# mstksg/tensor-ops

Hardware: AMD Instinct MI355X
Metric: gradTOp steps/sec (ffLayer MNIST 784->256->10) + gmul TFLOP/s vs roofline (higher is better)
Workload: dtype f32

## Files before the change

tensor-ops_amd/csrc/gemm_small.hip:

```cpp
#include "common.hpp"

namespace to {

typedef float f32x16 __attribute__((ext_vector_type(16)));

template <class S>
struct SmallArgsT {
  const S* A;
  const S* B;
  S* C;
  const S* Cin;
  int M, N, K;
  long a_sm, a_sk, b_sk, b_sn, c_sm;
  long a_sb, b_sb, c_sb;
  int a_vec, b_vec;
  unsigned a_bytes, b_bytes;
  int tiles_n;
  int tiles_m;
  int tile_order;
  int kper;
  S alpha, beta;
  const S* bias;
  const S* dact;
  int act;
  int dact_kind;
  S* rowsum;
  const S* rowsum_in;
  S rowsum_alpha;
  int rowsum_acc;
  int loss_rows;
  const S* target;
  S* loss_out;
  const S* tail_w;
// ... 6 lines not shown
};

#ifdef TOPS_AB_KNOBS
#define SM_STAMP(i) do { if (stamp_on) g.dbg[i] = wall_clock64(); } while (0)
#else
#define SM_STAMP(i) do { } while (0)
#endif


template <class G>
__device__ __forceinline__ void tile_of(const G& g, int bid, int& tile_m, int& tile_n) {
  if (g.tile_order) {
    const int T = g.tiles_m * g.tiles_n, x = bid & 7, q = T >> 3, r = T & 7;
    bid = (x < r ? x * (q + 1) : r * (q + 1) + (x - r) * q) + (bid >> 3);
  }
  if (g.tile_order == 2) {
    tile_n = bid / g.tiles_m;
    tile_m = bid - tile_n * g.tiles_m;
  } else {
    tile_m = bid / g.tiles_n;
    tile_n = bid - tile_m * g.tiles_n;
  }
}

__device__ __forceinline__ float tanh_s(float x) { return tanhf(x); }
__device__ __forceinline__ double tanh_s(double x) { return tanh(x); }
__device__ __forceinline__ float exp_s(float x) { return expf(x); }
__device__ __forceinline__ double exp_s(double x) { return exp(x); }
__device__ __forceinline__ float log_s(float x) { return logf(x); }
__device__ __forceinline__ double log_s(double x) { return log(x); }
__device__ __forceinline__ float max_s(float a, float b) { return fmaxf(a, b); }
__device__ __forceinline__ double max_s(double a, double b) { return fmax(a, b); }

template <class S, int AMODE, int BMODE, int NW, int TS, int ONESHOT = 0, bool EXT = false>
__device__ __forceinline__ void gemm_small_body(const SmallArgsT<S>& g, const int bid, const long bz, S* ext_lds = nullptr,
                                                const int tid_in = -1) {
  constexpr int ES = (int)sizeof(S);
  static_assert(ES == 4 || TS == 16, "the fp64 matrix instruction is 16x16x4");
  constexpr int KG = (TS == 32) ? 2 : 4;
  constexpr int NR = (TS == 32) ? 16 : 4;
  constexpr int CK = 4 * KG;
  typedef S accv __attribute__((ext_vector_type(NR)));
  S (*red)[NR][64];
  S (*rsum)[64];
  S* dzs;
  if constexpr (EXT) {
    red = reinterpret_cast<S (*)[NR][64]>(ext_lds);
    rsum = reinterpret_cast<S (*)[64]>(ext_lds + NW * NR * 64);
    dzs = ext_lds + NW * NR * 64 + NW * 64;
  } else {
    __shared__ S red_s[NW][NR][64];
    __shared__ S rsum_s[NW][64];
    __shared__ S dzs_s[TS == 16 ? 16 * 17 : 1];
    red = red_s;
    rsum = rsum_s;
    dzs = dzs_s;
  }
  const int tid = tid_in >= 0 ? tid_in : (int)threadIdx.x, lane = tid & 63, wave = tid >> 6;
  const int l31 = lane & (TS - 1), half = lane / TS;
#ifdef TOPS_AB_KNOBS
  const bool stamp_on = g.dbg && bid == 0 && tid == 0;
#endif
  SM_STAMP(0);
  int tile_m, tile_n;
  tile_of(g, bid, tile_m, tile_n);
  const long m = (long)tile_m * TS + l31, n = (long)tile_n * TS + l31;
  const bool mv = m < g.M, nv = n < g.N;
// ... 38 lines not shown
      d[0] = __hiloint2double((int)v.y, (int)v.x); d[1] = __hiloint2double((int)v.w, (int)v.z);
      d[2] = __hiloint2double((int)w.y, (int)w.x); d[3] = __hiloint2double((int)w.w, (int)w.z);
    }
  };
  auto load_stage = [&](S (&a)[ST][4], S (&b)[ST][4], int k0) {
#pragma unroll
    for (int c = 0; c < ST; ++c) {
      const int kb = k0 + CK * c + 4 * half;
      if (AMODE == 0 && g.a_vec) {
        ld4(ra, mv & (kb < kend), a_base + kb * ES, a[c]);
      } else {
#pragma unroll
        for (int j = 0; j < 4; ++j) a[c][j] = ld1(ra, sel(mv & (kb + j < kend), a_base + (kb + j) * a_sk4));
      }
      if (BMODE == 1 && g.b_vec) {
        ld4(rb, nv & (kb < kend), b_base + kb * ES, b[c]);
      } else {
#pragma unroll
        for (int j = 0; j < 4; ++j) b[c][j] = ld1(rb, sel(nv & (kb + j < kend), b_base + (kb + j) * b_sk4));
      }
    }
  };
  auto mma_stage = [&](const S (&a)[ST][4], const S (&b)[ST][4]) {
#pragma unroll
    for (int c = 0; c < ST; ++c)
#pragma unroll
      for (int j = 0; j < 4; ++j) {
        if constexpr (ES == 8) acc = __builtin_amdgcn_mfma_f64_16x16x4f64(a[c][j], b[c][j], acc, 0, 0, 0);
        else if constexpr (TS == 32) acc = __builtin_amdgcn_mfma_f32_32x32x2f32(a[c][j], b[c][j], acc, 0, 0, 0);
        else acc = __builtin_amdgcn_mfma_f32_16x16x4f32(a[c][j], b[c][j], acc, 0, 0, 0);
        asum += a[c][j];
      }
  };
  auto row16 = [&](int kg, int r) { return ES == 8 ? kg + 4 * r : 4 * kg + r; };
  constexpr int NRW = (NR + NW - 1) / NW;
  S* Cb = g.C + bz * g.c_sb;
  const S* Ci = g.Cin ? g.Cin + bz * g.c_sb : nullptr;
  const S* Hd = g.dact ? g.dact + bz * g.c_sb : nullptr;
  S pf_ci[NRW], pf_hd[NRW], pf_bias = S(0);
  {
    const long col = (long)tile_n * TS + l31;
    if (g.bias && col < g.N) pf_bias = g.bias[col];
#pragma unroll
    for (int i = 0; i < NRW; ++i) {
      const int r = wave + i * NW;
      const int lrow = (TS == 32) ? (r & 3) + 8 * (r >> 2) + 4 * half : row16(half, r);
      const long row = (long)tile_m * TS + lrow;
      const bool ok = r < NR && row < g.M && col < g.N;
      pf_ci[i] = (Ci && ok) ? Ci[row * g.c_sm + col] : S(0);
      pf_hd[i] = (Hd && ok) ? Hd[row * g.c_sm + col] : S(0);
    }
  }
  constexpr int SK = CK * ST;
  SM_STAMP(1);
  if constexpr (ONESHOT) {
    if (kbeg < kend) {
      load_stage(a0, b0, kbeg);
#ifdef TOPS_AB_KNOBS
      if (stamp_on) { SM_STAMP(2); __builtin_amdgcn_s_waitcnt(0x0F70); SM_STAMP(3); }
#endif
      mma_stage(a0, b0);
    }
  } else {
    S a1[ST][4], b1[ST][4];
    if (kbeg < kend) load_stage(a0, b0, kbeg);
    for (int k0 = kbeg; k0 < kend; k0 += 2 * SK) {
      if (k0 + SK < kend) load_stage(a1, b1, k0 + SK);
      mma_stage(a0, b0);
      if (k0 + SK < kend) {
        if (k0 + 2 * SK < kend) load_stage(a0, b0, k0 + 2 * SK);
        mma_stage(a1, b1);
      }
    }
  }

  S tl_bw[2][4], tl_hv[2][4];
  if constexpr (TS == 16) {
    if (g.loss_rows && g.tail_out) {
      const int l15 = lane & 15, kg = lane >> 4;
      const int ntiles = (g.tail_n + 15) / 16;
#pragma unroll
      for (int u = 0; u < 2; ++u) {
        const int t = wave + u * NW;
        const long col = (long)t * 16 + l15;
        const bool cv = t < ntiles && col < g.tail_n;
#pragma unroll
        for (int st = 0; st < 4; ++st) {
          const int k = 4 * st + kg;
          tl_bw[u][st] = (cv && k < g.N) ? g.tail_w[(long)k * g.tail_n + col] : S(0);
        }
#pragma unroll
        for (int r = 0; r < 4; ++r) {
          const long row = (long)tile_m * 16 + row16(kg, r);
          tl_hv[u][r] = (cv && row < g.M) ? g.tail_h[row * g.tail_n + col] : S(0);
// ... 91 lines not shown
        if (4 * st < g.N) {
          const S a = dzs[l15 * 17 + 4 * st + kg];
#pragma unroll
          for (int u = 0; u < 2; ++u) {
            if constexpr (ES == 8) acc2[u] = __builtin_amdgcn_mfma_f64_16x16x4f64(a, tl_bw[u][st], acc2[u], 0, 0, 0);
            else acc2[u] = __builtin_amdgcn_mfma_f32_16x16x4f32(a, tl_bw[u][st], acc2[u], 0, 0, 0);
          }
        }
      }
#pragma unroll
      for (int u = 0; u < 2; ++u) {
        const int t = wave + u * NW;
        const long col = (long)t * 16 + l15;
#pragma unroll
        for (int r = 0; r < 4; ++r) {
          const long row = (long)tile_m * 16 + row16(kg, r);
          if (t < ntiles && row < g.M && col < g.tail_n)
            g.tail_out[row * g.tail_n + col] = acc2[u][r] * tl_hv[u][r] * (S(1) - tl_hv[u][r]);
        }
      }
      SM_STAMP(7);
    }
  }
#ifdef TOPS_AB_KNOBS
  if (stamp_on) { __builtin_amdgcn_s_waitcnt(0); SM_STAMP(8); }
#endif
}

template <class S, int AMODE, int BMODE, int NW, int TS, int ONESHOT = 0>
__global__ __launch_bounds__(NW * 64) void gemm_small_kernel(SmallArgsT<S> g) {
  gemm_small_body<S, AMODE, BMODE, NW, TS, ONESHOT>(g, (int)blockIdx.x, (long)blockIdx.z);
}

template <class S, int A1, int B1, int NW1, int TS1, int OS1, int A2, int B2, int NW2, int TS2, int OS2>
__global__ __launch_bounds__((NW1 > NW2 ? NW1 : NW2) * 64) void gemm_small_pair_kernel(SmallArgsT<S> g1,
                                                                                         SmallArgsT<S> g2, int n1) {
  if ((int)blockIdx.x < n1) {
    if (NW1 < NW2 && (int)(threadIdx.x >> 6) >= NW1) return;
    gemm_small_body<S, A1, B1, NW1, TS1, OS1>(g1, (int)blockIdx.x, 0);
  } else {
    if (NW2 < NW1 && (int)(threadIdx.x >> 6) >= NW2) return;
    gemm_small_body<S, A2, B2, NW2, TS2, OS2>(g2, (int)blockIdx.x - n1, 0);
  }
}

struct ChainSync {
  unsigned* ctr;
  int* status;
  long long timeout;
  int dev;
};

__device__ __forceinline__ bool chain_barrier(const ChainSync& cs, int which, unsigned epoch) {
  __shared__ int ok;
  if (cs.dev == 1) {
    __syncthreads();
    return true;
  }
  if (cs.dev != 2) __builtin_amdgcn_fence(__ATOMIC_RELEASE, "agent");
  if (threadIdx.x == 0) ok = 1;
  __syncthreads();
  unsigned* flags = cs.ctr + which * 256;
  if (threadIdx.x == 0) __hip_atomic_store(flags + blockIdx.x, epoch, __ATOMIC_RELEASE, __HIP_MEMORY_SCOPE_AGENT);
  if (threadIdx.x < gridDim.x) {
    const long long t0 = wall_clock64();
    while (__hip_atomic_load(flags + threadIdx.x, __ATOMIC_RELAXED, __HIP_MEMORY_SCOPE_AGENT) < epoch) {
      if (wall_clock64() - t0 > cs.timeout) {
        ok = 0;
        *cs.status = 1 + which;
        break;
      }
      __builtin_amdgcn_s_sleep(1);
// ... 612 lines not shown
  c.mode = enable == 2 ? 2 : 1;
  c.status = g_seam_status_dev;
  static long long* dbg = [] {
    long long* p = nullptr;
    if (ab_getenv("TOPS_SEAM_STAMPS") && hipHostMalloc(&p, 8 * sizeof(long long), hipHostMallocMapped) == hipSuccess) {
      for (int i = 0; i < 8; ++i) p[i] = 0;
      static long long* keep = p;
      atexit([] {
        std::fprintf(stderr, "[seam] row block 0's head (us since its workgroup began): forward done %.2f, stores in L2 %.2f, "
                             "all tiles arrived %.2f, head done %.2f\n",
                     (keep[1] - keep[0]) * 0.01, (keep[2] - keep[0]) * 0.01, (keep[3] - keep[0]) * 0.01, (keep[4] - keep[0]) * 0.01);
      });
      return p;
    }
    return (long long*)nullptr;
  }();
  c.dbg = dbg;
  constexpr size_t lds = (16 * 16 * 64 + 16 * 64 + 16 * 17 + 16) * sizeof(float);
  launch_k(gemm_small_seam_kernel, dim3(T), dim3(1024), lds, s, c);
  TO_HIP(hipGetLastError());
  count_launch();
  return true;
}

void launch_gemm_small(const GemmProblem& p, hipStream_t s) {
  if (gemm_t32_applicable(p)) {
    launch_gemm_t32(p, s);
    return;
  }
  if (p.dtype == TO_F64) launch_small_t<double>(p, s);
  else launch_small_t<float>(p, s);
}

bool launch_gemm_small_pair(const GemmProblem& p1, const GemmProblem& p2, hipStream_t s) {
  static const int enable = [] { const char* e = ab_getenv("TOPS_SMALL_PAIR"); return e ? atoi(e) : 1; }();
  if (!enable || p1.dtype != p2.dtype || p1.batch != 1 || p2.batch != 1) return false;
  if (launch_gemm_t32_pair(p1, p2, s)) return true;
  if (!gemm_small_can(p1) || !gemm_small_can(p2)) return false;
  if (p1.dtype == TO_F64) {
    SmallArgsT<double> g1, g2;
    const SmallPlan c1 = plan_small<double>(p1, g1), c2 = plan_small<double>(p2, g2);
    if (!(c1.f64_t32 && c1.nw == 8 && c1.os == 1 && c1.amode == 1 && c1.bmode == 0)) return false;
    if (!(!c2.f64_t32 && c2.ts == 16 && c2.nw == 8 && c2.os == 8 && c2.amode == 1 && c2.bmode == 0)) return false;
    if (g1.loss_rows || g2.loss_rows) return false;
    const int n1 = (int)((p1.M + 31) / 32) * g1.tiles_n, n2 = (int)((p2.M + 15) / 16) * g2.tiles_n;
    launch_k((gemm_small_pair_f64_kernel<1, 0, 1, 0>), dim3(n1 + n2), dim3(512), 0, s, g1, g2, n1);
    TO_HIP(hipGetLastError());
    count_launch();
    return true;
  }
  SmallArgsT<float> g1, g2;
  const SmallPlan c1 = plan_small<float>(p1, g1), c2 = plan_small<float>(p2, g2);
#ifdef TOPS_AB_KNOBS
  g1.dbg = small_stamps(1);
  g2.dbg = small_stamps(3);
#endif
  if (!(c1.ts == 32 && c1.nw == 16 && c1.os == 8 && c1.amode == 1 && c1.bmode == 0)) return false;
  if (!(c2.ts == 16 && c2.nw == 8 && c2.os == 8 && c2.amode == 1 && c2.bmode == 0)) return false;
  if (g1.loss_rows || g2.loss_rows) return false;
  const int n1 = (int)((p1.M + 31) / 32) * g1.tiles_n, n2 = (int)((p2.M + 15) / 16) * g2.tiles_n;
  dim3 grid(n1 + n2), block(1024);
  launch_k((gemm_small_pair_kernel<float, 1, 0, 16, 32, 8, 1, 0, 8, 16, 8>), grid, block, 0, s, g1, g2, n1);
  TO_HIP(hipGetLastError());
  count_launch();
  return true;
}

}
```

tensor-ops_amd/csrc/gemm_t32.hip:

```cpp
#include <cstdio>
#include <type_traits>

#include "common.hpp"

namespace to {

typedef float f32x16 __attribute__((ext_vector_type(16)));
typedef float f32x4 __attribute__((ext_vector_type(4)));

struct T32Args {
  const float* A;
  const float* B;
  float* C;
  const float* Cin;
  const float* bias;
  const float* dact;
  float* rowsum;
  const float* rowsum_in;
  unsigned long long* dbg;
  long a_sx, b_sx;
  long c_sm;
  int M, N, K;
  int tiles_m, tiles_n;
  int gm, gn;
  int act, dact_kind;
  int rowsum_acc;
  int pd;
  float alpha, beta;
  float rowsum_alpha;
};

__device__ __attribute__((aligned(16))) float g_t32_zero[4] = {0.f, 0.f, 0.f, 0.f};

constexpr int T32_BK = 32, T32_NS = 2, T32_NW = 4;
constexpr int T32_CTR = 4096;
constexpr int T32_STAGE = 2 * 32 * T32_BK;
constexpr int T32_WAVE = T32_NS * T32_STAGE;

__device__ __forceinline__ bool t32_tile_of(int tiles_m, int tiles_n, int gm, int gn, int bid, int& tm, int& tn) {
  const int x = bid & 7, local = bid >> 3, xm = x / gn, xn = x - xm * gn;
  const int r0 = tiles_m * xm / gm, r1 = tiles_m * (xm + 1) / gm, c0 = tiles_n * xn / gn, c1 = tiles_n * (xn + 1) / gn;
  const int w = c1 - c0;
  if (w <= 0 || local >= (r1 - r0) * w) return false;
  tm = r0 + local / w;
  tn = c0 + local - (local / w) * w;
  return true;
}

__device__ __forceinline__ int t32_key(int x) { return (x >> 1) & 7; }

template <bool AKC, bool BKC, bool ARAG = false, bool WT = false>
__device__ __forceinline__ int gemm_t32_body(const T32Args& g, const int bid, float* smem) {
  static_assert(!ARAG || !AKC, "the dword form is for a row-contiguous A");
  constexpr int NA = ARAG ? 16 : 4, PER = NA + 4;
  const int tid = threadIdx.x, lane = tid & 63;
  const int wave = __builtin_amdgcn_readfirstlane(tid >> 6);
  const int l31 = lane & 31, half = lane >> 5;
  unsigned long long* const dbg = (g.dbg && tid == 0 && (bid == 0 || bid == (int)gridDim.x - 1)) ? g.dbg + (bid == 0 ? 0 : 8) : nullptr;
  auto stamp = [&](int i) { if (dbg) dbg[i] = __builtin_amdgcn_s_memrealtime(); };
  int tile_m, tile_n;
  if (!t32_tile_of(g.tiles_m, g.tiles_n, g.gm, g.gn, bid, tile_m, tile_n)) return -1;
  stamp(0);
  const int m0 = tile_m * 32, n0 = tile_n * 32;

  const int erow = tid >> 3, ec4 = (tid & 7) * 4;
  const long grow = m0 + erow, gcol = n0 + ec4;
  const bool evalid = grow < g.M && gcol < g.N;
  f32x4 pf_ci = {0.f, 0.f, 0.f, 0.f}, pf_hd = {0.f, 0.f, 0.f, 0.f}, pf_bias = {0.f, 0.f, 0.f, 0.f};
  if (evalid) {
    if (g.Cin) pf_ci = *reinterpret_cast<const f32x4*>(g.Cin + grow * g.c_sm + gcol);
    if (g.dact) pf_hd = *reinterpret_cast<const f32x4*>(g.dact + grow * g.c_sm + gcol);
    if (g.bias) pf_bias = *reinterpret_cast<const f32x4*>(g.bias + gcol);
  }

  const int U = (g.K + 15) / 16;
  const int k0 = (int)((long)U * wave / T32_NW) * 16;
  int k1 = (int)((long)U * (wave + 1) / T32_NW) * 16;
  if (k1 > g.K) k1 = g.K;
  const int nC = k1 > k0 ? (k1 - k0 + T32_BK - 1) / T32_BK : 0;

  typedef __attribute__((address_space(3))) void* lptr_t;
  float* wsm = smem + wave * T32_WAVE;
  const unsigned lds_w = __builtin_amdgcn_readfirstlane((unsigned)(unsigned long)(lptr_t)wsm);

  const int lr = lane >> 3, ls = lane & 7;
  unsigned oa[4], ob[4];
  bool xa_ok = true, xb_ok = true;
#pragma unroll
  for (int p = 0; p < 4; ++p) {
    if constexpr (AKC) {
      long x = m0 + 8 * p + lr;
      if (x >= g.M) x = g.M - 1;
      oa[p] = (unsigned)((x * g.a_sx + 4 * (ls ^ t32_key(8 * p + lr))) * 4);
    } else {
      oa[p] = (unsigned)(((long)(8 * p + lr) * g.a_sx + m0 + 4 * ls) * 4);
    }
    if constexpr (BKC) {
      long x = n0 + 8 * p + lr;
      if (x >= g.N) x = g.N - 1;
      ob[p] = (unsigned)((x * g.b_sx + 4 * (ls ^ t32_key(8 * p + lr))) * 4);
    } else {
      ob[p] = (unsigned)(((long)(8 * p + lr) * g.b_sx + n0 + 4 * ls) * 4);
    }
  }
  if constexpr (!AKC) xa_ok = m0 + 4 * ls + 3 < g.M;
  if constexpr (!BKC) xb_ok = n0 + 4 * ls + 3 < g.N;
  const bool interior = !ARAG && (AKC || m0 + 32 <= g.M) && (BKC || n0 + 32 <= g.N);
  const long step_a = AKC ? T32_BK * 4L : T32_BK * g.a_sx * 4L, step_b = BKC ? T32_BK * 4L : T32_BK * g.b_sx * 4L;
  const char* sa = reinterpret_cast<const char*>(g.A) + (AKC ? (long)k0 * 4 : (long)k0 * g.a_sx * 4);
  const char* sb = reinterpret_cast<const char*>(g.B) + (BKC ? (long)k0 * 4 : (long)k0 * g.b_sx * 4);

#define T32_DMA(OFF, BASE) asm volatile("global_load_lds_dwordx4 %0, %1 offset:0" ::"v"(OFF), "s"(BASE) : "memory")
#define T32_DMA_V(PTR) asm volatile("global_load_lds_dwordx4 %0, off offset:0" ::"v"(PTR) : "memory")
  const long a_sx_l = g.a_sx;
  const int M_l = g.M;
  auto issue = [&, a_sx_l, M_l](int c) {
    const int seq = c;
    const int kc = k0 + c * T32_BK;
    const unsigned st = lds_w + (unsigned)(seq % T32_NS) * (T32_STAGE * 4);
    const char* ba = sa + (long)c * step_a;
    const char* bb = sb + (long)c * step_b;
    const bool full = kc + T32_BK <= k1;
    if (full && interior) {
#pragma unroll
      for (int p = 0; p < 4; ++p) {
        asm volatile("s_mov_b32 m0, %0\n\ts_nop 0" ::"s"(st + p * 1024) : "memory");
        T32_DMA(oa[p], ba);
      }
#pragma unroll
      for (int p = 0; p < 4; ++p) {
        asm volatile("s_mov_b32 m0, %0\n\ts_nop 0" ::"s"(st + 4096 + p * 1024) : "memory");
        T32_DMA(ob[p], bb);
      }
    } else {
      const char* zero = reinterpret_cast<const char*>(g_t32_zero);
      if constexpr (ARAG) {
#pragma unroll
        for (int e = 0; e < 16; ++e) {
          const int kl = 2 * e + half;
          const bool ok = kc + kl < k1 && m0 + l31 < M_l;
          const char* src = ok ? ba + ((long)kl * a_sx_l + m0 + l31) * 4 : zero;
          asm volatile("s_mov_b32 m0, %0\n\ts_nop 0" ::"s"(st + e * 256) : "memory");
          asm volatile("global_load_lds_dword %0, off offset:0" ::"v"(src) : "memory");
        }
      } else {
#pragma unroll
        for (int p = 0; p < 4; ++p) {
          const bool ok = AKC ? (kc + 4 * (ls ^ t32_key(8 * p + lr)) < k1) : (kc + 8 * p + lr < k1 && xa_ok);
          const char* src = ok ? ba + oa[p] : zero;
          asm volatile("s_mov_b32 m0, %0\n\ts_nop 0" ::"s"(st + p * 1024) : "memory");
          T32_DMA_V(src);
        }
      }
#pragma unroll
      for (int p = 0; p < 4; ++p) {
        const bool ok = BKC ? (kc + 4 * (ls ^ t32_key(8 * p + lr)) < k1) : (kc + 8 * p + lr < k1 && xb_ok);
        const char* src = ok ? bb + ob[p] : zero;
        asm volatile("s_mov_b32 m0, %0\n\ts_nop 0" ::"s"(st + 4096 + p * 1024) : "memory");
        T32_DMA_V(src);
      }
    }
  };
#undef T32_DMA
#undef T32_DMA_V

  f32x16 acc;
#pragma unroll
  for (int r = 0; r < 16; ++r) acc[r] = 0.f;
  float asum = 0.f;
  const bool want_rs = g.rowsum != nullptr && tile_n == 0;

  const int PD = g.pd;
  const int pro = nC < PD ? nC : PD;
  for (int c = 0; c < pro; ++c) issue(c);
  stamp(1);

  auto wait_landed = [&](int c) {
    const int newer = (nC - 1 - c) < (PD - 1) ? (nC - 1 - c) : (PD - 1);
    static_assert(3 * PER <= 63, "vmcnt is six bits");
    if (newer >= 3) asm volatile("s_waitcnt vmcnt(%0)" ::"n"(3 * PER) : "memory");
    else if (newer == 2) asm volatile("s_waitcnt vmcnt(%0)" ::"n"(2 * PER) : "memory");
    else if (newer == 1) asm volatile("s_waitcnt vmcnt(%0)" ::"n"(PER) : "memory");
    else asm volatile("s_waitcnt vmcnt(0)" ::: "memory");
  };
  auto steps_of = [&](int c) { return (k1 - (k0 + c * T32_BK)) > 16 ? 4 : 2; };
  auto read_frags = [&](int c, float (&fa)[16], float (&fb)[16]) {
    const float* sp = wsm + (c % T32_NS) * T32_STAGE;
    const int nI = steps_of(c);
#pragma unroll
    for (int i = 0; i < 4; ++i) {
      if (i < nI) {
        if constexpr (AKC) {
          const f32x4 v = *reinterpret_cast<const f32x4*>(sp + l31 * 32 + 4 * ((2 * i + half) ^ t32_key(l31)));
          fa[4 * i] = v.x; fa[4 * i + 1] = v.y; fa[4 * i + 2] = v.z; fa[4 * i + 3] = v.w;
        } else {
#pragma unroll
          for (int j = 0; j < 4; ++j) fa[4 * i + j] = sp[(4 * (2 * i + half) + j) * 32 + l31];
        }
        if constexpr (BKC) {
          const f32x4 v = *reinterpret_cast<const f32x4*>(sp + 1024 + l31 * 32 + 4 * ((2 * i + half) ^ t32_key(l31)));
          fb[4 * i] = v.x; fb[4 * i + 1] = v.y; fb[4 * i + 2] = v.z; fb[4 * i + 3] = v.w;
        } else {
#pragma unroll
          for (int j = 0; j < 4; ++j) fb[4 * i + j] = sp[1024 + (4 * (2 * i + half) + j) * 32 + l31];
        }
      }
    }
  };
  auto mma = [&](int c, const float (&fa)[16], const float (&fb)[16]) {
    const int nI = steps_of(c);
#pragma unroll
    for (int i = 0; i < 4; ++i) {
      if (i < nI) {
#pragma unroll
        for (int j = 0; j < 4; ++j) {
          acc = __builtin_amdgcn_mfma_f32_32x32x2f32(fa[4 * i + j], fb[4 * i + j], acc, 0, 0, 0);
          if (want_rs) asum += fa[4 * i + j];
        }
      }
    }
  };
  float fa[16], fb[16];
  for (int c = 0; c < nC; ++c) {
    wait_landed(c);
    if (c == 0) stamp(2);
    read_frags(c, fa, fb);
    asm volatile("s_waitcnt lgkmcnt(0)" ::: "memory");
    __builtin_amdgcn_sched_barrier(0);
    if (c + PD < nC) issue(c + PD);
    __builtin_amdgcn_sched_barrier(0);
    mma(c, fa, fb);
  }
  asm volatile("s_waitcnt vmcnt(0)" ::: "memory");
  stamp(3);

#pragma unroll
  for (int r = 0; r < 16; ++r) wsm[((r & 3) + 8 * (r >> 2) + 4 * half) * 32 + l31] = acc[r];
  if (want_rs) wsm[1024 + lane] = asum;
  __syncthreads();
  stamp(4);
  f32x4 s = *reinterpret_cast<const f32x4*>(smem + erow * 32 + ec4);
#pragma unroll
  for (int w = 1; w < T32_NW; ++w) s += *reinterpret_cast<const f32x4*>(smem + w * T32_WAVE + erow * 32 + ec4);
  if (evalid) {
    f32x4 v = s * g.alpha;
    if (g.Cin) v += pf_ci * g.beta;
    if (g.bias) v += pf_bias;
    if (g.act == 1) {
      v.x = 1.f / (1.f + __expf(-v.x)); v.y = 1.f / (1.f + __expf(-v.y));
      v.z = 1.f / (1.f + __expf(-v.z)); v.w = 1.f / (1.f + __expf(-v.w));
    } else if (g.act == 2) {
      v.x = tanhf(v.x); v.y = tanhf(v.y); v.z = tanhf(v.z); v.w = tanhf(v.w);
    }
    if (g.dact) {
      if (g.dact_kind == 0) v *= pf_hd * (1.f - pf_hd);
      else v *= 1.f - pf_hd * pf_hd;
    }
    if constexpr (WT) {
      typedef unsigned int u32x4 __attribute__((ext_vector_type(4)));
      const u32x4 u = {__float_as_uint(v.x), __float_as_uint(v.y), __float_as_uint(v.z), __float_as_uint(v.w)};
      float* dst = g.C + grow * g.c_sm + gcol;
      asm volatile("global_store_dwordx4 %0, %1, off sc0 sc1" ::"v"(dst), "v"(u) : "memory");
    } else {
      *reinterpret_cast<f32x4*>(g.C + grow * g.c_sm + gcol) = v;
    }
  }
  if (want_rs && tid < 32) {
    const long m = m0 + tid;
    if (m < g.M) {
      float t = 0.f;
#pragma unroll
      for (int w = 0; w < T32_NW; ++w) t += smem[w * T32_WAVE + 1024 + tid] + smem[w * T32_WAVE + 1024 + 32 + tid];
      if (g.rowsum_acc) g.rowsum[m] = (g.rowsum_in ? g.rowsum_in[m] : g.rowsum[m]) + g.rowsum_alpha * t;
      else g.rowsum[m] = t;
    }
  }
  stamp(5);
  return tile_m;
}

struct T32HeadArgs {
  const float* W2;
  const float* bias2;
  const float* target;
  float* dz;
  float* loss_out;
  float* tail_out;
  unsigned* ctr;
  int* status;
  long w_sn, dz_sm;
  int N2, loss_rows;
  float alpha2;
};

__global__ __launch_bounds__(256) void gemm_t32_head_kernel(T32Args g, T32HeadArgs h) {
  extern __shared__ __attribute__((aligned(1024))) float t32_smem[];
  const int tid = threadIdx.x, lane = tid & 63;
  const int wave = __builtin_amdgcn_readfirstlane(tid >> 6);
  const unsigned long long t_entry = g.dbg ? __builtin_amdgcn_s_memrealtime() : 0ull;
  int tile_m, tile_n;
  if (!t32_tile_of(g.tiles_m, g.tiles_n, g.gm, g.gn, (int)blockIdx.x, tile_m, tile_n)) return;
  const long grow = (long)tile_m * 32 + 4 * tile_n + wave;
  const bool rv = grow < g.M;
  f32x4 w4[16];
#pragma unroll
// ... 74 lines not shown
    out_l = lv ? -2.f * e * sg * (1.f - sg) : 0.f;
    loss_l = lv ? e * e : 0.f;
  }
  if (rv) {
    if (lv) h.dz[grow * h.dz_sm + lane] = out_l;
    if (h.loss_out) {
      const float l = sum16(loss_l);
      if (lane == 0) h.loss_out[grow] = l;
    }
  }
  if (hd) hd[3] = __builtin_amdgcn_s_memrealtime();
  if (h.tail_out) {
    f32x4 a = {0.f, 0.f, 0.f, 0.f};
#pragma unroll
    for (int n = 0; n < 16; ++n)
      if (n < h.N2) {
        const float d = __shfl(out_l, n, 64);
        a += w4[n] * d;
      }
    if (rv) *reinterpret_cast<f32x4*>(h.tail_out + grow * 256 + 4 * lane) = a * h4 * (1.f - h4);
  }
  if (hd) hd[4] = __builtin_amdgcn_s_memrealtime();
  __syncthreads();
  if (tid == 0) {
    unsigned* leave = h.ctr + T32_CTR + tile_m;
    const unsigned seen = __hip_atomic_fetch_add(leave, 1u, __ATOMIC_RELAXED, __HIP_MEMORY_SCOPE_AGENT);
    if (seen == (unsigned)(g.tiles_n - 1)) {
      __hip_atomic_store(h.ctr + tile_m, 0u, __ATOMIC_RELAXED, __HIP_MEMORY_SCOPE_AGENT);
      __hip_atomic_store(leave, 0u, __ATOMIC_RELAXED, __HIP_MEMORY_SCOPE_AGENT);
    }
  }
}

template <bool AKC, bool BKC>
__global__ __launch_bounds__(256) void gemm_t32_kernel(T32Args g) {
  extern __shared__ __attribute__((aligned(1024))) float t32_smem[];
  gemm_t32_body<AKC, BKC>(g, (int)blockIdx.x, t32_smem);
}

template <bool ARAG2>
__global__ __launch_bounds__(256) void gemm_t32_pair_kernel(T32Args g1, T32Args g2, int n1) {
  extern __shared__ __attribute__((aligned(1024))) float t32_smem[];
  if ((int)blockIdx.x < n1) gemm_t32_body<false, false, false>(g1, (int)blockIdx.x, t32_smem);
  else gemm_t32_body<false, false, ARAG2>(g2, (int)blockIdx.x - n1, t32_smem);
}

static bool t32_fill(const GemmProblem& p, T32Args& g, bool& akc, bool& bkc, bool allow_ragged_a = false, bool* ragged_a = nullptr) {
  if (p.dtype != TO_F32 || p.batch != 1 || p.reduce_batch) return false;
  if (p.loss_rows || p.tail_out || p.loss_out) return false;
  akc = p.a_sk == 1 && p.K > 1;
  bkc = p.b_sk == 1 && p.K > 1;
  if (!akc && p.a_sm != 1) return false;
  if (!bkc && p.b_sn != 1) return false;
  if (p.K % 4 != 0 || p.N % 4 != 0) return false;
  const bool rag = !akc && (p.M % 4 != 0 || p.a_sk % 4 != 0 || (reinterpret_cast<uintptr_t>(p.A) & 15u));
  if (ragged_a) *ragged_a = rag;
  if (rag && !allow_ragged_a) return false;
  if (akc && p.a_sm % 4 != 0) return false;
  if (bkc && p.b_sn % 4 != 0) return false;
  if (!bkc && p.b_sk % 4 != 0) return false;
  if ((reinterpret_cast<uintptr_t>(p.A) & 3u) || ((akc || !rag) && (reinterpret_cast<uintptr_t>(p.A) & 15u))) return false;
  if ((reinterpret_cast<uintptr_t>(p.B) | reinterpret_cast<uintptr_t>(p.C)) & 15u) return false;
  if (p.c_sm % 4 != 0) return false;
  if (p.Cin && (reinterpret_cast<uintptr_t>(p.Cin) & 15u)) return false;
  if (p.dact && (reinterpret_cast<uintptr_t>(p.dact) & 15u)) return false;
  if (p.bias && (reinterpret_cast<uintptr_t>(p.bias) & 15u)) return false;
  if (p.beta != 0.0 && !p.Cin) return false;
  if (p.act > 2) return false;
  if ((p.M + 32) * std::max<int64_t>(p.a_sm, 1) * 4 + p.K * std::max<int64_t>(p.a_sk, 1) * 4 >= (1LL << 31)) return false;
  if ((p.N + 32) * std::max<int64_t>(p.b_sn, 1) * 4 + p.K * std::max<int64_t>(p.b_sk, 1) * 4 >= (1LL << 31)) return false;
// ... 35 lines not shown
          std::fprintf(stderr, "[t32] %s workgroup of the last launch, us since it began: prologue DMA issued %.2f, first chunk landed %.2f, K loop done %.2f, "
                               "partials met %.2f, done %.2f; began %.2f us after workgroup 0\n", w ? "last" : "first",
                       (k[1] - k[0]) * 0.01, (k[2] - k[0]) * 0.01, (k[3] - k[0]) * 0.01, (k[4] - k[0]) * 0.01, (k[5] - k[0]) * 0.01,
                       ((double)k[0] - (double)keep[0]) * 0.01);
        }
      });
    }
    return p;
  }();
  g.dbg = dbg;
  return true;
}

bool gemm_t32_applicable(const GemmProblem& p) {
  static const int enable = [] { const char* e = ab_getenv("TOPS_GEMM_T32"); return e ? atoi(e) : 1; }();
  if (!enable) return false;
  T32Args g;
  bool akc, bkc;
  if (!t32_fill(p, g, akc, bkc)) return false;
  const long tiles = (long)g.tiles_m * g.tiles_n;
  static const long max_tiles = [] { const char* e = ab_getenv("TOPS_T32_MAXTILES"); return e ? atol(e) : 512L; }();
  return tiles >= 96 && tiles <= max_tiles && p.K >= 256 && p.K <= 8192;
}

bool launch_gemm_t32_pair(const GemmProblem& p1, const GemmProblem& p2, hipStream_t s);

static long t32_grid(const T32Args& g) {
  const long rm = (g.tiles_m + g.gm - 1) / g.gm, rn = (g.tiles_n + g.gn - 1) / g.gn;
  return 8 * rm * rn;
}

static void t32_attr(const void* k) { TO_HIP(hipFuncSetAttribute(k, hipFuncAttributeMaxDynamicSharedMemorySize, T32_NW * T32_WAVE * 4)); }

void launch_gemm_t32(const GemmProblem& p, hipStream_t s) {
  T32Args g;
  bool akc, bkc;
  TO_CHECK(t32_fill(p, g, akc, bkc), TO_ERR_STATE, "launch_gemm_t32: not applicable");
  static bool attr = false;
  if (!attr) {
    t32_attr(reinterpret_cast<const void*>(gemm_t32_kernel<true, true>));
    t32_attr(reinterpret_cast<const void*>(gemm_t32_kernel<true, false>));
    t32_attr(reinterpret_cast<const void*>(gemm_t32_kernel<false, true>));
    t32_attr(reinterpret_cast<const void*>(gemm_t32_kernel<false, false>));
    attr = true;
  }
  const dim3 grid((unsigned)t32_grid(g)), block(256);
  const size_t lds = (size_t)T32_NW * T32_WAVE * 4;
  if (akc && bkc) launch_k(gemm_t32_kernel<true, true>, grid, block, lds, s, g);
  else if (akc) launch_k(gemm_t32_kernel<true, false>, grid, block, lds, s, g);
  else if (bkc) launch_k(gemm_t32_kernel<false, true>, grid, block, lds, s, g);
  else launch_k(gemm_t32_kernel<false, false>, grid, block, lds, s, g);
  TO_HIP(hipGetLastError());
  count_launch();
}

static unsigned* g_t32_ctr = nullptr;
static int *g_t32_status = nullptr, *g_t32_status_dev = nullptr;
static bool g_t32_head_off = false;
void gemm_t32_init() {
  if (g_t32_ctr) return;
  if (hipMalloc(&g_t32_ctr, 2 * T32_CTR * sizeof(unsigned)) != hipSuccess || hipMemset(g_t32_ctr, 0, 2 * T32_CTR * sizeof(unsigned)) != hipSuccess) {
    (void)hipGetLastError();
    g_t32_ctr = nullptr;
    return;
  }
  if (hipHostMalloc(&g_t32_status, sizeof(int), hipHostMallocMapped) == hipSuccess) {
    *g_t32_status = 0;
    if (hipHostGetDevicePointer(reinterpret_cast<void**>(&g_t32_status_dev), g_t32_status, 0) != hipSuccess) g_t32_status_dev = nullptr;
  }
  (void)hipGetLastError();
}
int gemm_t32_take_failure() {
  const int st = g_t32_status ? *g_t32_status : 0;
  if (st) {
    g_t32_head_off = true;
    *g_t32_status = 0;
    if (g_t32_ctr) (void)hipMemset(g_t32_ctr, 0, 2 * T32_CTR * sizeof(unsigned));
  }
  return st;
}

bool launch_gemm_t32_head(const GemmProblem& pf, const GemmProblem& ph, hipStream_t s) {
  static const int enable = [] { const char* e = getenv("TOPS_STEP_SEAM"); return e ? atoi(e) : 0; }();
  if (enable != 3 || !g_t32_ctr || !g_t32_status_dev || g_t32_head_off) return false;
// ... 68 lines not shown
```

Measured before the change: 39410.

## Split one-shot small GEMM into staged parts and add 8-wave t32 variant

```diff
diff --git a/tensor-ops_amd/csrc/gemm_small.hip b/tensor-ops_amd/csrc/gemm_small.hip
--- a/tensor-ops_amd/csrc/gemm_small.hip
+++ b/tensor-ops_amd/csrc/gemm_small.hip
@@ -1,4 +1,6 @@
 #include "common.hpp"
+
+#include <type_traits>
 
 namespace to {
 
@@ -71,7 +73,7 @@
 __device__ __forceinline__ float max_s(float a, float b) { return fmaxf(a, b); }
 __device__ __forceinline__ double max_s(double a, double b) { return fmax(a, b); }
 
-template <class S, int AMODE, int BMODE, int NW, int TS, int ONESHOT = 0, bool EXT = false>
+template <class S, int AMODE, int BMODE, int NW, int TS, int ONESHOT = 0, bool EXT = false, int PARTS = 0, bool STAG = false>
 __device__ __forceinline__ void gemm_small_body(const SmallArgsT<S>& g, const int bid, const long bz, S* ext_lds = nullptr,
                                                 const int tid_in = -1) {
   constexpr int ES = (int)sizeof(S);
@@ -176,6 +178,44 @@
         asum += a[c][j];
       }
   };
+  constexpr int CP = PARTS ? ST / PARTS : ST;
+  static_assert(PARTS == 0 || (ONESHOT && ST % PARTS == 0), "PARTS divides the one-shot batch");
+  auto load_part = [&](auto part, int k0) {
+    constexpr int p = decltype(part)::value;
+#pragma unroll
+    for (int c = p * CP; c < (p + 1) * CP; ++c) {
+      const int kb = k0 + CK * c + 4 * half;
+      if (AMODE == 0 && g.a_vec) {
+        ld4(ra, mv & (kb < kend), a_base + kb * ES, a0[c]);
+      } else {
+#pragma unroll
+        for (int j = 0; j < 4; ++j) a0[c][j] = ld1(ra, sel(mv & (kb + j < kend), a_base + (kb + j) * a_sk4));
+      }
+      if (BMODE == 1 && g.b_vec) {
+        ld4(rb, nv & (kb < kend), b_base + kb * ES, b0[c]);
+      } else {
+#pragma unroll
+        for (int j = 0; j < 4; ++j) b0[c][j] = ld1(rb, sel(nv & (kb + j < kend), b_base + (kb + j) * b_sk4));
+      }
+      __builtin_amdgcn_sched_barrier(0);
+    }
+  };
+  auto mma_part = [&](auto part) {
+    constexpr int p = decltype(part)::value;
+#pragma unroll
+    for (int c = p * CP; c < (p + 1) * CP; ++c) {
+#pragma unroll
+      for (int j = 0; j < 4; ++j) {
+        if constexpr (ES == 8) acc = __builtin_amdgcn_mfma_f64_16x16x4f64(a0[c][j], b0[c][j], acc, 0, 0, 0);
+        else if constexpr (TS == 32) acc = __builtin_amdgcn_mfma_f32_32x32x2f32(a0[c][j], b0[c][j], acc, 0, 0, 0);
+        else acc = __builtin_amdgcn_mfma_f32_16x16x4f32(a0[c][j], b0[c][j], acc, 0, 0, 0);
+      }
+      __builtin_amdgcn_sched_barrier(0);
+#pragma unroll
+      for (int j = 0; j < 4; ++j) asum += a0[c][j];
+      __builtin_amdgcn_sched_barrier(0);
+    }
+  };
   auto row16 = [&](int kg, int r) { return ES == 8 ? kg + 4 * r : 4 * kg + r; };
   constexpr int NRW = (NR + NW - 1) / NW;
   S* Cb = g.C + bz * g.c_sb;
@@ -198,12 +238,43 @@
   constexpr int SK = CK * ST;
   SM_STAMP(1);
   if constexpr (ONESHOT) {
-    if (kbeg < kend) {
-      load_stage(a0, b0, kbeg);
+    if constexpr (PARTS == 0) {
+      if (kbeg < kend) {
+        load_stage(a0, b0, kbeg);
 #ifdef TOPS_AB_KNOBS
-      if (stamp_on) { SM_STAMP(2); __builtin_amdgcn_s_waitcnt(0x0F70); SM_STAMP(3); }
+        if (stamp_on) { SM_STAMP(2); __builtin_amdgcn_s_waitcnt(0x0F70); SM_STAMP(3); }
 #endif
-      mma_stage(a0, b0);
+        mma_stage(a0, b0);
+      }
+    } else if (kbeg < kend) {
+      if constexpr (STAG) {
+        const int lvl = __builtin_amdgcn_readfirstlane(wave) >> 2;
+        if (lvl == 0) __builtin_amdgcn_s_setprio(3);
+        else if (lvl == 1) __builtin_amdgcn_s_setprio(2);
+        else if (lvl == 2) __builtin_amdgcn_s_setprio(1);
+      }
+      load_part(std::integral_constant<int, 0>{}, kbeg);
+      auto stage = [&](auto part) {
+        constexpr int p = decltype(part)::value;
+        if constexpr (p + 1 < PARTS) load_part(std::integral_constant<int, p + 1>{}, kbeg);
+        if constexpr (STAG && p == (PARTS >= 2 ? PARTS - 2 : 0)) __builtin_amdgcn_s_setprio(0);
+        __builtin_amdgcn_sched_barrier(0);
+        if constexpr (p == 0) SM_STAMP(2);
+        mma_part(part);
+        __builtin_amdgcn_sched_barrier(0);
+        if constexpr (p == 0) SM_STAMP(3);
+      };
+      stage(std::integral_constant<int, 0>{});
+      if constexpr (PARTS > 1) stage(std::integral_constant<int, 1>{});
+      if constexpr (PARTS > 2) stage(std::integral_constant<int, 2>{});
+      if constexpr (PARTS > 3) stage(std::integral_constant<int, 3>{});
+      if constexpr (PARTS > 4) {
+        stage(std::integral_constant<int, 4>{});
+        stage(std::integral_constant<int, 5>{});
+        stage(std::integral_constant<int, 6>{});
+        stage(std::integral_constant<int, 7>{});
+      }
+      static_assert(PARTS == 1 || PARTS == 2 || PARTS == 4 || PARTS == 8, "one, two, four or eight parts");
     }
   } else {
     S a1[ST][4], b1[ST][4];
@@ -361,12 +432,12 @@
   gemm_small_body<S, AMODE, BMODE, NW, TS, ONESHOT>(g, (int)blockIdx.x, (long)blockIdx.z);
 }
 
-template <class S, int A1, int B1, int NW1, int TS1, int OS1, int A2, int B2, int NW2, int TS2, int OS2>
+template <class S, int A1, int B1, int NW1, int TS1, int OS1, int A2, int B2, int NW2, int TS2, int OS2, int P1 = 0, bool STAG1 = false>
 __global__ __launch_bounds__((NW1 > NW2 ? NW1 : NW2) * 64) void gemm_small_pair_kernel(SmallArgsT<S> g1,
                                                                                          SmallArgsT<S> g2, int n1) {
   if ((int)blockIdx.x < n1) {
     if (NW1 < NW2 && (int)(threadIdx.x >> 6) >= NW1) return;
-    gemm_small_body<S, A1, B1, NW1, TS1, OS1>(g1, (int)blockIdx.x, 0);
+    gemm_small_body<S, A1, B1, NW1, TS1, OS1, false, P1, STAG1>(g1, (int)blockIdx.x, 0);
   } else {
     if (NW2 < NW1 && (int)(threadIdx.x >> 6) >= NW2) return;
     gemm_small_body<S, A2, B2, NW2, TS2, OS2>(g2, (int)blockIdx.x - n1, 0);
@@ -1045,6 +1116,9 @@
   else launch_small_t<float>(p, s);
 }
 
+constexpr int SMALL_PAIR_PARTS = 8;
+constexpr bool SMALL_PAIR_STAG = false;
+
 bool launch_gemm_small_pair(const GemmProblem& p1, const GemmProblem& p2, hipStream_t s) {
   static const int enable = [] { const char* e = ab_getenv("TOPS_SMALL_PAIR"); return e ? atoi(e) : 1; }();
   if (!enable || p1.dtype != p2.dtype || p1.batch != 1 || p2.batch != 1) return false;
@@ -1073,7 +1147,26 @@
   if (g1.loss_rows || g2.loss_rows) return false;
   const int n1 = (int)((p1.M + 31) / 32) * g1.tiles_n, n2 = (int)((p2.M + 15) / 16) * g2.tiles_n;
   dim3 grid(n1 + n2), block(1024);
-  launch_k((gemm_small_pair_kernel<float, 1, 0, 16, 32, 8, 1, 0, 8, 16, 8>), grid, block, 0, s, g1, g2, n1);
+#define TOPS_PAIR(P, ST) launch_k((gemm_small_pair_kernel<float, 1, 0, 16, 32, 8, 1, 0, 8, 16, 8, P, ST>), grid, block, 0, s, g1, g2, n1)
+#ifdef TOPS_AB_KNOBS
+  static const int parts = [] { const char* e = ab_getenv("TOPS_SMALL_PARTS"); return e ? atoi(e) : SMALL_PAIR_PARTS; }();
+  static const int stag = [] { const char* e = ab_getenv("TOPS_SMALL_STAGGER"); return e ? atoi(e) : (int)SMALL_PAIR_STAG; }();
+  switch (parts * 2 + (stag ? 1 : 0)) {
+    case 0: TOPS_PAIR(0, false); break;
+    case 2: TOPS_PAIR(1, false); break;
+    case 3: TOPS_PAIR(1, true); break;
+    case 4: TOPS_PAIR(2, false); break;
+    case 5: TOPS_PAIR(2, true); break;
+    case 8: TOPS_PAIR(4, false); break;
+    case 9: TOPS_PAIR(4, true); break;
+    case 16: TOPS_PAIR(8, false); break;
+    case 17: TOPS_PAIR(8, true); break;
+    default: TO_CHECK(false, TO_ERR_ARG, "TOPS_SMALL_PARTS is 0, 1, 2, 4 or 8 (TOPS_SMALL_STAGGER needs parts >= 1)");
+  }
+#else
+  TOPS_PAIR(SMALL_PAIR_PARTS, SMALL_PAIR_STAG);
+#endif
+#undef TOPS_PAIR
   TO_HIP(hipGetLastError());
   count_launch();
   return true;
diff --git a/tensor-ops_amd/csrc/gemm_t32.hip b/tensor-ops_amd/csrc/gemm_t32.hip
--- a/tensor-ops_amd/csrc/gemm_t32.hip
+++ b/tensor-ops_amd/csrc/gemm_t32.hip
@@ -49,8 +49,10 @@
 
 __device__ __forceinline__ int t32_key(int x) { return (x >> 1) & 7; }
 
-template <bool AKC, bool BKC, bool ARAG = false, bool WT = false>
+template <bool AKC, bool BKC, bool ARAG = false, bool WT = false, int NW = T32_NW, int NS = T32_NS, bool EARLY = false>
 __device__ __forceinline__ int gemm_t32_body(const T32Args& g, const int bid, float* smem) {
+  constexpr int WAVE_F = NS * T32_STAGE;
+  static_assert(WAVE_F >= 1024 + 64, "a wave's stage memory holds its partial tile and its row sums");
   static_assert(!ARAG || !AKC, "the dword form is for a row-contiguous A");
   constexpr int NA = ARAG ? 16 : 4, PER = NA + 4;
   const int tid = threadIdx.x, lane = tid & 63;
@@ -65,22 +67,25 @@
 
   const int erow = tid >> 3, ec4 = (tid & 7) * 4;
   const long grow = m0 + erow, gcol = n0 + ec4;
-  const bool evalid = grow < g.M && gcol < g.N;
+  const bool evalid = (NW == 4 || tid < 256) && grow < g.M && gcol < g.N;
   f32x4 pf_ci = {0.f, 0.f, 0.f, 0.f}, pf_hd = {0.f, 0.f, 0.f, 0.f}, pf_bias = {0.f, 0.f, 0.f, 0.f};
-  if (evalid) {
-    if (g.Cin) pf_ci = *reinterpret_cast<const f32x4*>(g.Cin + grow * g.c_sm + gcol);
-    if (g.dact) pf_hd = *reinterpret_cast<const f32x4*>(g.dact + grow * g.c_sm + gcol);
-    if (g.bias) pf_bias = *reinterpret_cast<const f32x4*>(g.bias + gcol);
-  }
+  auto prefetch_epilogue = [&] {
+    if (evalid) {
+      if (g.Cin) pf_ci = *reinterpret_cast<const f32x4*>(g.Cin + grow * g.c_sm + gcol);
+      if (g.dact) pf_hd = *reinterpret_cast<const f32x4*>(g.dact + grow * g.c_sm + gcol);
+      if (g.bias) pf_bias = *reinterpret_cast<const f32x4*>(g.bias + gcol);
+    }
+  };
+  if constexpr (!EARLY) prefetch_epilogue();
 
   const int U = (g.K + 15) / 16;
-  const int k0 = (int)((long)U * wave / T32_NW) * 16;
-  int k1 = (int)((long)U * (wave + 1) / T32_NW) * 16;
+  const int k0 = (int)((long)U * wave / NW) * 16;
+  int k1 = (int)((long)U * (wave + 1) / NW) * 16;
   if (k1 > g.K) k1 = g.K;
   const int nC = k1 > k0 ? (k1 - k0 + T32_BK - 1) / T32_BK : 0;
 
   typedef __attribute__((address_space(3))) void* lptr_t;
-  float* wsm = smem + wave * T32_WAVE;
+  float* wsm = smem + wave * WAVE_F;
   const unsigned lds_w = __builtin_amdgcn_readfirstlane((unsigned)(unsigned long)(lptr_t)wsm);
 
   const int lr = lane >> 3, ls = lane & 7;
@@ -117,7 +122,7 @@
   auto issue = [&, a_sx_l, M_l](int c) {
     const int seq = c;
     const int kc = k0 + c * T32_BK;
-    const unsigned st = lds_w + (unsigned)(seq % T32_NS) * (T32_STAGE * 4);
+    const unsigned st = lds_w + (unsigned)(seq % NS) * (T32_STAGE * 4);
     const char* ba = sa + (long)c * step_a;
     const char* bb = sb + (long)c * step_b;
     const bool full = kc + T32_BK <= k1;
@@ -170,9 +175,17 @@
   float asum = 0.f;
   const bool want_rs = g.rowsum != nullptr && tile_n == 0;
 
-  const int PD = g.pd;
+  const int PD = g.pd < NS ? g.pd : NS;
   const int pro = nC < PD ? nC : PD;
-  for (int c = 0; c < pro; ++c) issue(c);
+  if constexpr (EARLY) {
+    if (pro > 0) issue(0);
+    __builtin_amdgcn_sched_barrier(0);
+    prefetch_epilogue();
+    __builtin_amdgcn_sched_barrier(0);
+    for (int c = 1; c < pro; ++c) issue(c);
+  } else {
+    for (int c = 0; c < pro; ++c) issue(c);
+  }
   stamp(1);
 
   auto wait_landed = [&](int c) {
@@ -185,7 +198,7 @@
   };
   auto steps_of = [&](int c) { return (k1 - (k0 + c * T32_BK)) > 16 ? 4 : 2; };
   auto read_frags = [&](int c, float (&fa)[16], float (&fb)[16]) {
-    const float* sp = wsm + (c % T32_NS) * T32_STAGE;
+    const float* sp = wsm + (c % NS) * T32_STAGE;
     const int nI = steps_of(c);
 #pragma unroll
     for (int i = 0; i < 4; ++i) {
@@ -239,9 +252,12 @@
   if (want_rs) wsm[1024 + lane] = asum;
   __syncthreads();
   stamp(4);
-  f32x4 s = *reinterpret_cast<const f32x4*>(smem + erow * 32 + ec4);
-#pragma unroll
-  for (int w = 1; w < T32_NW; ++w) s += *reinterpret_cast<const f32x4*>(smem + w * T32_WAVE + erow * 32 + ec4);
+  f32x4 s = {0.f, 0.f, 0.f, 0.f};
+  if (NW == 4 || tid < 256) {
+    s = *reinterpret_cast<const f32x4*>(smem + erow * 32 + ec4);
+#pragma unroll
+    for (int w = 1; w < NW; ++w) s += *reinterpret_cast<const f32x4*>(smem + w * WAVE_F + erow * 32 + ec4);
+  }
   if (evalid) {
     f32x4 v = s * g.alpha;
     if (g.Cin) v += pf_ci * g.beta;
@@ -270,7 +286,7 @@
     if (m < g.M) {
       float t = 0.f;
 #pragma unroll
-      for (int w = 0; w < T32_NW; ++w) t += smem[w * T32_WAVE + 1024 + tid] + smem[w * T32_WAVE + 1024 + 32 + tid];
+      for (int w = 0; w < NW; ++w) t += smem[w * WAVE_F + 1024 + tid] + smem[w * WAVE_F + 1024 + 32 + tid];
       if (g.rowsum_acc) g.rowsum[m] = (g.rowsum_in ? g.rowsum_in[m] : g.rowsum[m]) + g.rowsum_alpha * t;
       else g.rowsum[m] = t;
     }
@@ -411,10 +427,10 @@
   }
 }
 
-template <bool AKC, bool BKC>
-__global__ __launch_bounds__(256) void gemm_t32_kernel(T32Args g) {
+template <bool AKC, bool BKC, int NW = T32_NW, int NS = T32_NS, bool EARLY = false>
+__global__ __launch_bounds__(NW * 64) void gemm_t32_kernel(T32Args g) {
   extern __shared__ __attribute__((aligned(1024))) float t32_smem[];
-  gemm_t32_body<AKC, BKC>(g, (int)blockIdx.x, t32_smem);
+  gemm_t32_body<AKC, BKC, false, false, NW, NS, EARLY>(g, (int)blockIdx.x, t32_smem);
 }
 
 template <bool ARAG2>
@@ -516,24 +532,50 @@
 
 static void t32_attr(const void* k) { TO_HIP(hipFuncSetAttribute(k, hipFuncAttributeMaxDynamicSharedMemorySize, T32_NW * T32_WAVE * 4)); }
 
+constexpr int T32_W8_DEFAULT = 1;
+constexpr int T32_W8_NS = 1;
+constexpr bool T32_EARLY = true;
+
+template <int NW, int NS, bool EARLY>
+static void t32_launch_nw(const T32Args& g, bool akc, bool bkc, hipStream_t s) {
+  constexpr size_t lds = (size_t)NW * NS * T32_STAGE * 4;
+  static bool attr = false;
+  if (!attr) {
+    TO_HIP(hipFuncSetAttribute(reinterpret_cast<const void*>(gemm_t32_kernel<true, true, NW, NS, EARLY>), hipFuncAttributeMaxDynamicSharedMemorySize, (int)lds));
+    TO_HIP(hipFuncSetAttribute(reinterpret_cast<const void*>(gemm_t32_kernel<true, false, NW, NS, EARLY>), hipFuncAttributeMaxDynamicSharedMemorySize, (int)lds));
+    TO_HIP(hipFuncSetAttribute(reinterpret_cast<const void*>(gemm_t32_kernel<false, true, NW, NS, EARLY>), hipFuncAttributeMaxDynamicSharedMemorySize, (int)lds));
+    TO_HIP(hipFuncSetAttribute(reinterpret_cast<const void*>(gemm_t32_kernel<false, false, NW, NS, EARLY>), hipFuncAttributeMaxDynamicSharedMemorySize, (int)lds));
+    attr = true;
+  }
+  const dim3 grid((unsigned)t32_grid(g)), block(NW * 64);
+  if (akc && bkc) launch_k((gemm_t32_kernel<true, true, NW, NS, EARLY>), grid, block, lds, s, g);
+  else if (akc) launch_k((gemm_t32_kernel<true, false, NW, NS, EARLY>), grid, block, lds, s, g);
+  else if (bkc) launch_k((gemm_t32_kernel<false, true, NW, NS, EARLY>), grid, block, lds, s, g);
+  else launch_k((gemm_t32_kernel<false, false, NW, NS, EARLY>), grid, block, lds, s, g);
+}
+
 void launch_gemm_t32(const GemmProblem& p, hipStream_t s) {
   T32Args g;
   bool akc, bkc;
   TO_CHECK(t32_fill(p, g, akc, bkc), TO_ERR_STATE, "launch_gemm_t32: not applicable");
-  static bool attr = false;
-  if (!attr) {
-    t32_attr(reinterpret_cast<const void*>(gemm_t32_kernel<true, true>));
-    t32_attr(reinterpret_cast<const void*>(gemm_t32_kernel<true, false>));
-    t32_attr(reinterpret_cast<const void*>(gemm_t32_kernel<false, true>));
-    t32_attr(reinterpret_cast<const void*>(gemm_t32_kernel<false, false>));
-    attr = true;
-  }
-  const dim3 grid((unsigned)t32_grid(g)), block(256);
-  const size_t lds = (size_t)T32_NW * T32_WAVE * 4;
-  if (akc && bkc) launch_k(gemm_t32_kernel<true, true>, grid, block, lds, s, g);
-  else if (akc) launch_k(gemm_t32_kernel<true, false>, grid, block, lds, s, g);
-  else if (bkc) launch_k(gemm_t32_kernel<false, true>, grid, block, lds, s, g);
-  else launch_k(gemm_t32_kernel<false, false>, grid, block, lds, s, g);
+  static const int cus = [] { hipDeviceProp_t pr; int d = 0; return (hipGetDevice(&d) == hipSuccess && hipGetDeviceProperties(&pr, d) == hipSuccess) ? pr.multiProcessorCount : 0; }();
+  static const int waves = [] { const char* e = ab_getenv("TOPS_T32_WAVES"); return e ? atoi(e) : (T32_W8_DEFAULT ? 8 : 4); }();
+  const bool w8 = waves == 8 && t32_grid(g) <= cus;
+#ifdef TOPS_AB_KNOBS
+  static const int w8_ns = [] { const char* e = ab_getenv("TOPS_T32_W8_NS"); return e ? atoi(e) : T32_W8_NS; }();
+  static const int early = [] { const char* e = ab_getenv("TOPS_T32_EARLY"); return e ? atoi(e) : (int)T32_EARLY; }();
+  switch ((w8 ? (w8_ns == 1 ? 2 : 4) : 0) + (early ? 1 : 0)) {
+    case 0: t32_launch_nw<T32_NW, T32_NS, false>(g, akc, bkc, s); break;
+    case 1: t32_launch_nw<T32_NW, T32_NS, true>(g, akc, bkc, s); break;
+    case 2: t32_launch_nw<8, 1, false>(g, akc, bkc, s); break;
+    case 3: t32_launch_nw<8, 1, true>(g, akc, bkc, s); break;
+    case 4: t32_launch_nw<8, 2, false>(g, akc, bkc, s); break;
+    default: t32_launch_nw<8, 2, true>(g, akc, bkc, s); break;
+  }
+#else
+  if (w8) t32_launch_nw<8, T32_W8_NS, T32_EARLY>(g, akc, bkc, s);
+  else t32_launch_nw<T32_NW, T32_NS, T32_EARLY>(g, akc, bkc, s);
+#endif
   TO_HIP(hipGetLastError());
   count_launch();
 }
```

Measured after the change: 41840 (median of 6 runs). 1.06x the previous value.
